# ielym/fastvision

Hardware: AMD Instinct MI355X
Metric: images/sec (640×640, bs=32/GPU) YOLOv3 train step, 1/2/4/8 MI355X (higher is better)
Workload: dtype bf16

## Files before the change

### fastvision_amd/csrc/conv_igemm.hip

```cpp
#include <stddef.h>
#include <stdlib.h>

#include "common.h"

namespace {

enum { EPI_STATS = 0, EPI_PLAIN = 1, EPI_HEAD = 2, EPI_BNACT = 3, EPI_BNB = 4 };
constexpr int MAX_TAPS = 10;

struct IgemmParams {
    const void* in;
    const void* wt;
    void* out;
    float* stats;
    int acc_rep, bnb_rep, ax_rep;
    long long* stats_acc;
    const float* bias;
    const float* scale;
    int act;
    const float* shift;
    int M, N, C;
    int OW, OHW;
    FastDiv div_ow, div_ohw;
    int in_img, in_row;
// ... 17 lines not shown
    const float *ax_scale, *ax_shift;
    int ax_pad, ax_res_pad, ax_H, ax_W;
    long long* ax_acc;
    long long* ax_zero;
    const float *ax_gamma, *ax_beta;
    float *ax_rm, *ax_rv;
    long long* ax_nbt;
    float ax_momentum, ax_eps;
    BnN ax_n;
    float *ax_save_mean, *ax_save_rstd, *ax_scale_out, *ax_shift_out;
    long long* stamps;
    int stamp_rows;
    int pt_tx, pt_ty, pt_H, pt_W;
    int pt_tiles, pt_tpb;
    FastDiv pt_div_tx, pt_div_img;
};

struct BnbCoef {
    float sc[8], sh[8], mu[8], rs[8];
};
__device__ __forceinline__ void bnb_load(const IgemmParams& p, int n, BnbCoef& k) {
#pragma unroll
    for (int e = 0; e < 8; ++e) {
        int c = n + e;
        c = c < p.N ? c : p.N - 1;
        c = c >= p.bnb_C ? c - p.bnb_C : c;
        k.sc[e] = p.bnb_scale[c]; k.sh[e] = p.bnb_shift[c]; k.mu[e] = p.bnb_mean[c]; k.rs[e] = p.bnb_rstd[c];
    }
}
template <int BN, int NT>
__device__ __forceinline__ float bnb_coef_at(const IgemmParams& p, int i, int n0) {
// ... 169 lines not shown
__device__ __forceinline__ void foreach_acc(Acc<float>& acc, int lane, F&& f) {
    const int r = lane & 31, h = lane >> 5;
#pragma unroll
    for (int mt = 0; mt < 2; ++mt)
#pragma unroll
        for (int nt = 0; nt < 2; ++nt)
#pragma unroll
            for (int e = 0; e < 16; ++e) f(mt * 32 + (e & 3) + 8 * (e >> 2) + 4 * h, nt * 32 + r, nt, acc.a[mt][nt][e]);
}

template <int N>
__device__ __forceinline__ void wait_vmcnt() {
    asm volatile("s_waitcnt vmcnt(%0)" ::"n"(N) : "memory");
}

template <typename T, int BM, int BN, int EPI, int NSTAGE, bool AX = false>
__global__ __launch_bounds__((BM / 64) * (BN / 64) * 64) void igemm_kernel(const IgemmParams p) {
    static_assert(!AX || (sizeof(T) == 2 && EPI == EPI_STATS), "the produced-operand form is the bf16 training forward of a 1x1 layer");
    constexpr int EPC = 16 / (int)sizeof(T);
    constexpr int BK = 8 * EPC;
    constexpr int WN = BN / 64;
    constexpr int NW = (BM / 64) * WN;
    constexpr int NT = NW * 64;
    static_assert(NW % 2 == 0, "the source swizzle assumes an even wave count");
    constexpr int A_BYTES = BM * 128, B_BYTES = BN * 128, STAGE = A_BYTES + B_BYTES;
    constexpr int A_ITERS = BM / (8 * NW), B_ITERS = BN / (8 * NW);
    constexpr bool IS_BF16 = sizeof(T) == 2;
    extern __shared__ __attribute__((aligned(16))) char smem[];

    const int tid = threadIdx.x, lane = tid & 63, w = tid >> 6;
    const int wr = w / WN, wc = w % WN;
    auto stamp = [&](int i) {
        if (p.stamps && tid == 0 && (int)blockIdx.x < p.stamp_rows) p.stamps[(int64_t)blockIdx.x * 8 + i] = wall_clock64();
    };
    stamp(0);

    const int nwg = gridDim.x, bid = blockIdx.x;
    const int xcd = bid & 7, xq = nwg >> 3, xr = nwg & 7;
    const int logical = (xcd < xr ? xcd * (xq + 1) : xr * (xq + 1) + (xcd - xr) * xq) + (bid >> 3);
    const int mblk = logical / p.nblocks, nblk = logical - mblk * p.nblocks;
    const int m0 = mblk * BM, n0 = nblk * BN;

    const T* a_ptr[A_ITERS];
    const T* b_ptr[B_ITERS];
    const int lrow = lane >> 3;
    const int sw = ((w & 1) << 2) + (lane >> 4);
    const int chunk = (lane & 7) ^ sw;
    const int tapsel = chunk >> 2;
    const int sub = p.halfrow ? (chunk & 3) : chunk;
#pragma unroll
    for (int i = 0; i < A_ITERS; ++i) {
        int m = m0 + (i * NW + w) * 8 + lrow;
        m = m < p.M ? m : p.M - 1;
        const uint32_t b = fd_div((uint32_t)m, p.div_ohw);
        const uint32_t rem = (uint32_t)m - b * (uint32_t)p.OHW;
        const uint32_t oy = fd_div(rem, p.div_ow);
// ... 7 lines not shown
        n = n < p.N ? n : p.N - 1;
        b_ptr[i] = (const T*)p.wt + (int64_t)n * p.C + sub * EPC;
    }

    constexpr bool USE_KTAB = BN >= 128;
    constexpr int COEF_BYTES = (EPI == EPI_BNB && IS_BF16 && BN >= 128) ? 4 * BN * 4 : 0;
    float* coef_tab = (float*)(smem + NSTAGE * STAGE);
    int* ktab = (int*)(smem + NSTAGE * STAGE + COEF_BYTES);
    constexpr int COEF_PER_THREAD = COEF_BYTES > 0 ? 4 * BN / NT : 0;
    float coef_v[COEF_PER_THREAD > 0 ? COEF_PER_THREAD : 1];
    if constexpr (COEF_BYTES > 0) {
#pragma unroll
        for (int j = 0; j < COEF_PER_THREAD; ++j) coef_v[j] = bnb_coef_at<BN, NT>(p, tid + j * NT, n0);
    }
    if constexpr (USE_KTAB) {
        const int nent = p.halfrow ? 2 * p.ktiles : p.ktiles;
        for (int e = tid; e < nent; e += NT) {
            int t, kk;
            if (p.halfrow) { t = e; kk = 0; }
            else if (p.ktaps) { kk = e / p.ktaps; t = e - kk * p.ktaps; }
            else { t = e / p.kt_per_tap; kk = e - t * p.kt_per_tap; }
            int tp = 0, tw = 0;
#pragma unroll
            for (int i = 0; i < MAX_TAPS; ++i)
                if (i == t) { tp = p.tap_pix[i]; tw = p.tap_w[i]; }
            ktab[2 * e] = tp * p.C + kk * BK;
            ktab[2 * e + 1] = tw * p.N * p.C + kk * BK;
        }
        __syncthreads();
    }
    stamp(6);
    int ld_tap = 0, ld_kk = 0;
    auto load_tile = [&](int kt, int stage) {
        char* sA = smem + stage * STAGE;
        char* sB = sA + A_BYTES;
        int aoff, boff;
        if constexpr (USE_KTAB) {
            const int e = p.halfrow ? 2 * kt + tapsel : kt;
            aoff = ktab[2 * e];
            boff = ktab[2 * e + 1];
        } else {
            const int t = p.halfrow ? ld_tap + tapsel : ld_tap;
            int tp = 0, tw = 0;
#pragma unroll
            for (int i = 0; i < MAX_TAPS; ++i)
                if (i == t) { tp = p.tap_pix[i]; tw = p.tap_w[i]; }
            aoff = tp * p.C + ld_kk * BK;
            boff = tw * p.N * p.C + ld_kk * BK;
            if (p.halfrow) ld_tap += 2;
            else if (++ld_kk == p.kt_per_tap) { ld_kk = 0; ++ld_tap; }
        }
#pragma unroll
        for (int i = 0; i < A_ITERS; ++i)
            __builtin_amdgcn_global_load_lds(GLB_PTR(a_ptr[i] + aoff), LDS_PTR(sA + (i * NW + w) * 1024), 16, 0, 0);
#pragma unroll
        for (int i = 0; i < B_ITERS; ++i)
            __builtin_amdgcn_global_load_lds(GLB_PTR(b_ptr[i] + boff), LDS_PTR(sB + (i * NW + w) * 1024), 16, 0, 0);
    };

    bf16x8 y_pre[8], a_pre[8];
    constexpr bool PREFETCH = (EPI == EPI_BNB || EPI == EPI_PLAIN) && sizeof(T) == 2;
// ... 1 lines not shown
        constexpr int CPR = BN / 8, RSTEP = NT / CPR;
        static_assert(BM * CPR / NT == 8, "the prefetch covers the whole store loop");
        const int cc = tid % CPR, r0 = tid / CPR;
        const int n = n0 + cc * 8;
#pragma unroll
        for (int j = 0; j < 8; ++j) {
            const int m = m0 + r0 + j * RSTEP;
            int64_t oi = 0;
            if (n < p.N && m < p.M) {
                int64_t pixel = m;
                if (!p.out_dense) {
                    const uint32_t b = fd_div((uint32_t)m, p.div_ohw);
                    const uint32_t rem = (uint32_t)m - b * (uint32_t)p.OHW;
                    const uint32_t oy = fd_div(rem, p.div_ow);
                    const uint32_t ox = rem - oy * (uint32_t)p.OW;
                    pixel = (int64_t)b * p.out_img + (int64_t)(oy * p.osy + p.ooy) * p.out_row + (ox * p.osx + p.oox);
                }
                oi = pixel * p.out_pitch + n;
            }
            if constexpr (EPI == EPI_BNB) y_pre[j] = ld_stream((const bf16_t*)p.bnb_y + oi);
            if (p.addend != nullptr) a_pre[j] = ld_stream((const bf16_t*)p.addend + oi);
        }
    }

    Acc<T> acc;
    if constexpr (sizeof(T) == 2) {
#pragma unroll
        for (int i = 0; i < 4; ++i)
#pragma unroll
            for (int j = 0; j < 4; ++j) acc.a[i][j] = f32x4{0.f, 0.f, 0.f, 0.f};
    } else {
// ... 51 lines not shown
        constexpr int S = decltype(set_tag)::value;
#pragma unroll
        for (int i = 0; i < A_ITERS; ++i) {
            ax_ry[S][i] = *(const bf16x8*)((const bf16_t*)p.ax_y + ax_yo[i] + kt * BK);
            if (ax_has_res) ax_rr[S][i] = *(const bf16x8*)((const bf16_t*)p.ax_res + ax_ro[i] + kt * BK);
        }
        if constexpr (!AXT) {
            const int c0 = kt * BK + chunk * 8;
            ax_csc[0] = *(const f32x4*)(p.ax_scale + c0); ax_csc[1] = *(const f32x4*)(p.ax_scale + c0 + 4);
            ax_csh[0] = *(const f32x4*)(p.ax_shift + c0); ax_csh[1] = *(const f32x4*)(p.ax_shift + c0 + 4);
        }
    };
    auto ax_step = [&](int kt, auto set_tag) {
        constexpr int S = decltype(set_tag)::value;
        if constexpr (AXS == 2) {
            if (kt + 1 < p.ktiles) {
                ax_load_raw(kt + 1, std::integral_constant<int, S ^ 1>{});
                if (ax_has_res) wait_vmcnt<2 * A_ITERS>();
                else wait_vmcnt<A_ITERS>();
            } else {
                wait_vmcnt<0>();
            }
        } else {
            wait_vmcnt<0>();
        }
        __builtin_amdgcn_sched_barrier(0);
        const uint32_t sAw = (uint32_t)(size_t)LDS_PTR(smem + st_cur * STAGE);
        f32x4 ax_sc[2], ax_sh[2];
        if constexpr (!AXT) {
            ax_sc[0] = ax_csc[0]; ax_sc[1] = ax_csc[1]; ax_sh[0] = ax_csh[0]; ax_sh[1] = ax_csh[1];
        } else {
// ... 29 lines not shown
                    if (f & 8u) {
                        *(bf16x8*)(q - zrow) = zero;
                        if (f & 2u) *(bf16x8*)(q - zrow - p.C) = zero;
                        if (f & 4u) *(bf16x8*)(q - zrow + p.C) = zero;
                    }
                    if (f & 16u) {
                        *(bf16x8*)(q + zrow) = zero;
                        if (f & 2u) *(bf16x8*)(q + zrow - p.C) = zero;
                        if (f & 4u) *(bf16x8*)(q + zrow + p.C) = zero;
                    }
                }
            }
        }
        asm volatile("s_waitcnt lgkmcnt(0)" ::: "memory");
        __builtin_amdgcn_s_barrier();
        if (kt + 1 < p.ktiles) {
            ax_issue_b(kt + 1, st_cur ^ 1);
            if constexpr (AXS == 1) ax_load_raw(kt + 1, std::integral_constant<int, 0>{});
        }
    };
    if constexpr (AX) {
        const int zp = p.ax_pad, rp = p.ax_res_pad;
        const uint32_t zW = (uint32_t)(p.ax_W + 2 * zp), zHW = (uint32_t)(p.ax_H + 2 * zp) * zW;
        const uint32_t rW = (uint32_t)(p.ax_W + 2 * rp), rHW = (uint32_t)(p.ax_H + 2 * rp) * rW;
#pragma unroll
        for (int i = 0; i < A_ITERS; ++i) {
            int m = m0 + (i * NW + w) * 8 + lrow;
            const bool live = m < p.M;
            m = live ? m : p.M - 1;
            const uint32_t b = fd_div((uint32_t)m, p.div_ohw);
            const uint32_t rem = (uint32_t)m - b * (uint32_t)p.OHW;
// ... 5 lines not shown
            ax_fl[i] = (live ? 1u : 0u) | (zp > 0 && live ? ((ox == 0 ? 2u : 0u) | (ox == (uint32_t)p.ax_W - 1 ? 4u : 0u) | (oy == 0 ? 8u : 0u) |
                                                           (oy == (uint32_t)p.ax_H - 1 ? 16u : 0u)) : 0u);
        }
        ax_load_raw(0, std::integral_constant<int, 0>{});
        if constexpr (AXT) {
            for (int c = tid; c < p.C; c += NT) ax_coef(c, logical == 0, ax_tab[c], ax_tab[p.C + c]);
            __syncthreads();
        }
        if (AXT && p.ax_acc != nullptr && logical == 0) {
            if (tid == 0 && p.ax_nbt) *p.ax_nbt += 1;
            fx_zero(p.ax_zero, p.C, p.ax_rep, tid, NT);
        }
        ax_issue_b(0, 0);
    } else {
        load_tile(0, 0);
        if (p.ktiles > 1) load_tile(1, 1);
    }
    stamp(1);
    for (int kt = 0; kt < p.ktiles; ++kt) {
        if constexpr (AX) {
            if (AXS == 1 || (kt & 1) == 0) ax_step(kt, std::integral_constant<int, 0>{});
            else ax_step(kt, std::integral_constant<int, AXS - 1>{});
            if (kt == 0) stamp(2);
        } else {
        if (kt == 0 && p.ktiles > 1) wait_vmcnt<LPT>();
        else wait_vmcnt<0>();
        __builtin_amdgcn_s_barrier();
        if (kt == 0) stamp(2);
        if (kt >= 1 && kt + 1 < p.ktiles) load_tile(kt + 1, st_cur ^ 1);
        }
        const char* sA = smem + st_cur * STAGE;
        const char* sB = sA + A_BYTES;
        st_cur ^= 1;
        if constexpr (IS_BF16) {
            const int r = lane & 15, g = lane >> 4, sr = (r >> 1) & 7;
            const char* pa = sA + (wr * 64 + r) * 128;
            const char* pb = sB + (wc * 64 + r) * 128;
#pragma unroll
            for (int ks = 0; ks < 2; ++ks) {
                const int co = ((ks * 4 + g) ^ sr) << 4;
                bf16x8 af[4], bfr[4];
#pragma unroll
                for (int t = 0; t < 4; ++t) {
                    af[t] = *(const bf16x8*)(pa + t * 16 * 128 + co);
// ... 111 lines not shown
                        if (p.stats_acc != nullptr) fx_atomic_add(fx_replica(p.stats_acc, p.N, p.acc_rep), p.N, which, n0 + col, s);
                        else *(p.stats + ((int64_t)mblk * 2 + which) * p.N + n0 + col) = s;
                    }
                }
                __syncthreads();
            }
        }
    }

    auto out_pixel = [&](int m) -> int64_t {
        if (p.out_dense) return m;
        const uint32_t b = fd_div((uint32_t)m, p.div_ohw);
        const uint32_t rem = (uint32_t)m - b * (uint32_t)p.OHW;
        const uint32_t oy = fd_div(rem, p.div_ow);
        const uint32_t ox = rem - oy * (uint32_t)p.OW;
        return (int64_t)b * p.out_img + (int64_t)(oy * p.osy + p.ooy) * p.out_row + (ox * p.osx + p.oox);
    };

    if constexpr (EPI == EPI_HEAD) {
        float* out = (float*)p.out;
        foreach_acc(acc, lane, [&](int row, int col, int, float v) {
            const int m = m0 + wrow0 + row, n = n0 + wcol0 + col;
            if (m < p.M && n < p.N) out[(int64_t)m * p.out_pitch + n] = v + p.bias[n];
        });
    } else if constexpr (!IS_BF16) {
        float* out = (float*)p.out;
        int64_t pix_cache = -1;
        int m_cache = -1;
        constexpr bool bnb = EPI == EPI_BNB;
        float b1[2] = {0.f, 0.f}, b2[2] = {0.f, 0.f}, ksc[2], ksh[2], kmu[2], krs[2];
        if constexpr (bnb) {
// ... 38 lines not shown
                    if (lane < 32) {
                        red[(0 * WMc + wr) * BN + wcol0 + i * 32 + lane] = b1[i];
                        red[(1 * WMc + wr) * BN + wcol0 + i * 32 + lane] = b2[i];
                    }
                }
                __syncthreads();
                if (w < BN / 32) {
                    const int which = lane >> 5, col = w * 32 + (lane & 31);
                    float t = 0.f;
#pragma unroll
                    for (int k = 0; k < WMc; ++k) t += red[(which * WMc + k) * BN + col];
                    const int n = n0 + col;
                    const int sub = n >= p.bnb_C ? 1 : 0, per = p.N > p.bnb_C ? 2 : 1;
                    if (n < p.N) {
                        if (p.bnb_acc != nullptr) fx_atomic_add(fx_replica(p.bnb_acc, p.bnb_C, p.bnb_rep), p.bnb_C, which, n - sub * p.bnb_C, t);
                        else *(p.bnb_part + (((int64_t)(p.bnb_row0 + mblk) * per + sub) * 2 + which) * p.bnb_C + (n - sub * p.bnb_C)) = t;
                    }
                }
            }
        }
    } else {
        constexpr int PITCH = BN * 2 + 16;
        if constexpr (EPI == EPI_BNB && COEF_BYTES == 0) {
            coef_tab = (float*)(smem + BM * PITCH);
            static_assert(4 * BN <= NT || EPI != EPI_BNB || COEF_BYTES > 0, "one table entry per thread");
            if (tid < 4 * BN) coef_v[0] = bnb_coef_at<BN, NT>(p, tid, n0);
        }
        {
            const int r = lane & 15, g = lane >> 4;
#pragma unroll
            for (int mt = 0; mt < 4; ++mt)
// ... 1 lines not shown
                for (int nt = 0; nt < 4; ++nt) {
                    f32x4 v = acc.a[mt][nt];
                    const int col = wcol0 + nt * 16 + 4 * g;
                    if constexpr (EPI == EPI_BNACT) {
#pragma unroll
                        for (int j = 0; j < 4; ++j) v[j] = bnact_f(p, v[j], n0 + col + j < p.N ? n0 + col + j : p.N - 1);
                    }
                    *(u32x2*)(smem + (wrow0 + mt * 16 + r) * PITCH + col * 2) = u32x2{cvt_pk_bf16(v[0], v[1]), cvt_pk_bf16(v[2], v[3])};
                }
        }
        if constexpr (EPI == EPI_BNB && COEF_BYTES == 0) {
            if (tid < 4 * BN) coef_tab[tid] = coef_v[0];
        }
        __syncthreads();
        stamp(4);
        store_tile_bf16<EPI, BM, BN, NT, PITCH>(p, smem, tid, n0, mblk, [&](int row) { const int m = m0 + row; return m < p.M ? out_pixel(m) : (int64_t)-1; },
                                                EPI == EPI_BNB ? y_pre : nullptr, PREFETCH ? a_pre : nullptr, coef_tab);
    }
    if constexpr (AX) {

    }
    stamp(5);
}

template <typename T, int BM, int BN, int EPI, int NSTAGE, bool AX = false>
int launch_one(const IgemmParams& p, hipStream_t s) {
    const int mblocks = cdiv(p.M, BM);
    IgemmParams q = p;
    q.nblocks = cdiv(p.N, BN);
    static const bool stamp_tiles = [] { const char* e = getenv("FVA_STAMP_IGEMM"); return e && atoi(e) != 0; }();
    q.stamps = stamp_tiles ? fva_debug_stamps_ptr() : nullptr;
    q.stamp_rows = stamp_tiles ? fva_debug_stamps_rows() : 0;
    constexpr int KTAB_MAX = 16384;
    const int nent = (p.halfrow ? 2 : 1) * p.ktiles;
    if (BN >= 128 && nent * 8 > KTAB_MAX) return fva_fail(FVA_ERR_ARG, "igemm: %d k-tiles exceed the offset table (%d)", p.ktiles, KTAB_MAX / 8);
    const int ktab_bytes = BN >= 128 ? (nent * 8 > 4096 ? (nent * 8 + 255) & ~255 : 4096) : 0;
    constexpr int coef_bytes = (EPI == EPI_BNB && sizeof(T) == 2 && BN >= 128) ? 4 * BN * 4 : 0;
    const int smem = NSTAGE * (BM + BN) * 128 + ktab_bytes + coef_bytes;
    static bool attr_done = false;
    if (!attr_done) {
        (void)hipFuncSetAttribute((const void*)igemm_kernel<T, BM, BN, EPI, NSTAGE, AX>, hipFuncAttributeMaxDynamicSharedMemorySize,
                                  NSTAGE * (BM + BN) * 128 + (BN >= 128 ? KTAB_MAX : 0) + coef_bytes);
        attr_done = true;
    }
    hipLaunchKernelGGL((igemm_kernel<T, BM, BN, EPI, NSTAGE, AX>), dim3(mblocks * q.nblocks), dim3((BM / 64) * (BN / 64) * 64), smem, s, q);
    FVA_LAUNCH_CHECK("igemm_kernel");
    fva_note_kernel(AX ? (BM == 128 ? "igemm128ax" : "igemm256x64ax") : (BM == 128 ? "igemm128" : "igemm256x64"));
    return FVA_OK;
}


struct PconvGeom {
    static constexpr int PH = 10, PW = 34, PW_RCP = 1928;
    static constexpr int OY = 8, OX = 32;
    static constexpr int TH = 8, TW_LOG2 = 5;
    static constexpr int NA = 4, NGRP = 4;
    static constexpr int MIN_CS = 32;
    static constexpr bool STATS = true, BNB_LOOPS = true;
    static constexpr const char *LABEL = "pconv", *KERNEL = "pconv_kernel";
    static __device__ __forceinline__ int frag_pix(int w, int a, int r16) { return (2 * w + (a >> 1)) * PW + (a & 1) * 16 + r16; }
// ... 299 lines not shown
    p.pt_ty = cdiv(H, G::TH);
    p.pt_div_tx = make_fastdiv(p.pt_tx);
    p.pt_div_img = make_fastdiv(p.pt_tx * p.pt_ty);
    for (int t = 0; t < 9; ++t) p.tap_w[t] = flip ? 8 - t : t;
    return G::template launch_form<EPI>(p, patch_tiles<G>(B, H, W), s);
}

struct Igemm8Diag {
    long long* stamps;
    int stamp_rows;
};

#ifndef FVA_EPI_STAMPS
#define FVA_EPI_STAMPS 0
#endif
template <int EPI>
__global__ __launch_bounds__(512) void igemm8_kernel(const IgemmParams p, const Igemm8Diag sk) {
    constexpr int MT = 8;
    constexpr int WM = 16 * MT;
    constexpr int BM = 2 * WM, BN = 256, NT = 512, BK = 64;
    constexpr int HALF = 128 * 128, BUF = 4 * HALF;
    constexpr int EPI_BYTES = BM * (BN * 2 + 16);
    constexpr int TAB0 = EPI_BYTES > 2 * BUF ? EPI_BYTES : 2 * BUF;
    extern __shared__ __attribute__((aligned(16))) char smem[];
    const int tid = threadIdx.x, lane = tid & 63, w = tid >> 6;
    const int wr = w >> 2, wc = w & 3;
    auto stamp = [&](int i) {
        if (sk.stamps && tid == 0 && (int)blockIdx.x < sk.stamp_rows) {
            sk.stamps[(int64_t)blockIdx.x * 8 + i] = wall_clock64();
            sk.stamps[(int64_t)blockIdx.x * 8 + 4 + i] = clock64();
        }
    };
#if !FVA_EPI_STAMPS
    stamp(0);
#endif

    const int nwg = gridDim.x, bid = blockIdx.x;
    const int xcd = bid & 7, xq = nwg >> 3, xr = nwg & 7;
    const int logical = (xcd < xr ? xcd * (xq + 1) : xr * (xq + 1) + (xcd - xr) * xq) + (bid >> 3);
    const int KT = p.ktiles;

    int* ktab = (int*)(smem + TAB0);
    for (int e = tid; e < KT; e += NT) {
        int t, kk;
        if (p.ktaps) { kk = e / p.ktaps; t = e - kk * p.ktaps; }
        else { t = e / p.kt_per_tap; kk = e - t * p.kt_per_tap; }
        int tp = 0, tw = 0;
#pragma unroll
        for (int i = 0; i < MAX_TAPS; ++i)
            if (i == t) { tp = p.tap_pix[i]; tw = p.tap_w[i]; }
        ktab[2 * e] = tp * p.C + kk * BK;
        ktab[2 * e + 1] = tw * p.N * p.C + kk * BK;
    }

    const int lrow = lane >> 3;
    const int chunk = (lane & 7) ^ (((w & 1) << 2) + (lane >> 4));
    const int r = lane & 15, g = lane >> 4, sr = (r >> 1) & 7;
    const int co0 = (g ^ sr) << 4, co1 = ((4 + g) ^ sr) << 4;
    const int a_row = (wr * 64 + r) * 128, b_row = (wc * 32 + r) * 128;

    {
        const int tile = logical, kt0 = 0, kt1 = KT;
        const int mblk = tile / p.nblocks, nblk = tile - mblk * p.nblocks;
        const int m0 = mblk * BM, n0 = nblk * BN;
        __syncthreads();
        float* coef_tab = (float*)(smem + TAB0 + 4096);
        if constexpr (EPI == EPI_BNB) bnb_fill_lds<BN, NT>(p, coef_tab, tid, n0);

        uint32_t a_off[2][2], b_off[2][2];
#pragma unroll
        for (int h = 0; h < 2; ++h)
#pragma unroll
            for (int i = 0; i < 2; ++i) {
                const int rh = (i * 8 + w) * 8 + lrow;
                int m = m0 + (rh >> 6) * WM + h * 64 + (rh & 63);
                m = m < p.M ? m : p.M - 1;
                const uint32_t b = fd_div((uint32_t)m, p.div_ohw);
                const uint32_t rem = (uint32_t)m - b * (uint32_t)p.OHW;
                const uint32_t oy = fd_div(rem, p.div_ow);
// ... 154 lines not shown
                    if (n0 + col < p.N) {
                        if (p.stats_acc != nullptr) fx_atomic_add(fx_replica(p.stats_acc, p.N, p.acc_rep), p.N, which, n0 + col, s);
                        else *(p.stats + ((int64_t)mblk * 2 + which) * p.N + n0 + col) = s;
                    }
                }
                __syncthreads();
            }
        }

        auto out_pixel = [&](int m) -> int64_t {
            if (p.out_dense) return m;
            const uint32_t b = fd_div((uint32_t)m, p.div_ohw);
            const uint32_t rem = (uint32_t)m - b * (uint32_t)p.OHW;
            const uint32_t oy = fd_div(rem, p.div_ow);
            const uint32_t ox = rem - oy * (uint32_t)p.OW;
            return (int64_t)b * p.out_img + (int64_t)(oy * p.osy + p.ooy) * p.out_row + (ox * p.osx + p.oox);
        };
        constexpr int PITCH = BN * 2 + 16;
#if FVA_EPI_STAMPS
        stamp(1);
#endif
#pragma unroll
        for (int mi = 0; mi < MT; ++mi)
#pragma unroll
            for (int ni = 0; ni < 4; ++ni) {
                f32x4 v = acc[mi][ni];
                if constexpr (EPI == EPI_BNACT) {
#pragma unroll
                    for (int j = 0; j < 4; ++j) v[j] = bnact_f(p, v[j], n0 + col_e + ni * 16 + j);
                }
                *(u32x2*)(smem + (row_e + mi * 16) * PITCH + (col_e + ni * 16) * 2) = u32x2{cvt_pk_bf16(v[0], v[1]), cvt_pk_bf16(v[2], v[3])};
            }
        __syncthreads();
#if FVA_EPI_STAMPS
        stamp(2);
#endif
        store_tile_bf16<EPI, BM, BN, NT, PITCH>(p, smem, tid_e, n0, mblk, [&](int row) { const int m = m0 + row; return m < p.M ? out_pixel(m) : (int64_t)-1; },
                                                nullptr, nullptr, EPI == EPI_BNB ? coef_tab : nullptr);
    }
    stamp(3);
}

constexpr int IGEMM8_SMEM = 256 * (256 * 2 + 16) + 4096 + 4096;

inline bool igemm8_enabled() {
    static bool v = [] {
        const char* e = getenv("FVA_IGEMM8");
        return !e || atoi(e) != 0;
    }();
    return v;
}
inline bool use_igemm8(int dtype, int64_t M, int N, int C, int ntaps, int64_t in_pixels) {
    if (!igemm8_enabled() || dtype != FVA_BF16 || N % 256 || C % 64) return false;
    if (in_pixels * C * 2 >= (1ll << 31) || (int64_t)(ntaps + 1) * N * C * 2 >= (1ll << 31)) return false;
    const int64_t ktiles = (int64_t)ntaps * (C / 64), tiles = (int64_t)cdiv(M, 256) * (N / 256);
    if (ktiles > 496 || ktiles < 8) return false;
    if (tiles < 128) return false;
    static const int min_kt = [] { const char* e = getenv("FVA_IGEMM8_MINKT"); return e ? atoi(e) : 16; }();
    return ktiles >= min_kt || tiles <= 256;
}

long long* g_stamps = nullptr;
int g_stamp_rows = 0;

template <int EPI>
int launch_igemm8(const IgemmParams& p, hipStream_t s) {
    IgemmParams q = p;
    q.nblocks = p.N / 256;
    const int tiles = cdiv(p.M, 256) * q.nblocks;
    static bool attr_done = false;
    if (!attr_done) {
        (void)hipFuncSetAttribute((const void*)igemm8_kernel<EPI>, hipFuncAttributeMaxDynamicSharedMemorySize, IGEMM8_SMEM);
        attr_done = true;
    }
    Igemm8Diag sk{};
    sk.stamps = g_stamps;
    sk.stamp_rows = g_stamp_rows;
    hipLaunchKernelGGL((igemm8_kernel<EPI>), dim3(tiles), dim3(512), IGEMM8_SMEM, s, q, sk);
    fva_note_kernel("igemm8");
    FVA_LAUNCH_CHECK("igemm8_kernel");
    return FVA_OK;
}

inline bool wide_tile(int N) { return N >= 128; }

inline int tile_bm(int , int , int N) { return wide_tile(N) ? 128 : 256; }

template <int EPI>
int launch_igemm(int dtype, const IgemmParams& p, hipStream_t s) {
    if (dtype == FVA_BF16) {
        if constexpr (EPI != EPI_HEAD) {
            if (!p.halfrow && use_igemm8(dtype, p.M, p.N, p.C, p.ktiles / p.kt_per_tap, (int64_t)(p.M / p.OHW + 1) * p.in_img))
                return launch_igemm8<EPI>(p, s);
        }
        return wide_tile(p.N) ? launch_one<bf16_t, 128, 128, EPI, 2>(p, s) : launch_one<bf16_t, 256, 64, EPI, 2>(p, s);
    }
    return wide_tile(p.N) ? launch_one<float, 128, 128, EPI, 2>(p, s) : launch_one<float, 256, 64, EPI, 2>(p, s);
}

int check_desc(const fva_conv_desc* d, const char* who) {
    if (!d) return fva_fail(FVA_ERR_ARG, "%s: null descriptor", who);
    if (d->dtype != FVA_F32 && d->dtype != FVA_BF16) return fva_fail(FVA_ERR_ARG, "%s: bad dtype %d", who, d->dtype);
    if (!((d->ksize == 1 && d->stride == 1) || (d->ksize == 3 && (d->stride == 1 || d->stride == 2))))
        return fva_fail(FVA_ERR_ARG, "%s: unsupported ksize/stride %d/%d", who, d->ksize, d->stride);
    if (d->B <= 0 || d->H <= 0 || d->W <= 0 || d->Cin <= 0 || d->Cout <= 0)
        return fva_fail(FVA_ERR_ARG, "%s: non-positive size", who);
    if (d->stride == 2 && ((d->H | d->W) & 1)) return fva_fail(FVA_ERR_ARG, "%s: stride 2 needs even H, W", who);
    if (d->in_pad < d->ksize / 2) return fva_fail(FVA_ERR_ARG, "%s: in_pad %d < %d", who, d->in_pad, d->ksize / 2);
    if ((int64_t)d->B * (d->H + 2) * (d->W + 2) >= (1ll << 31)) return fva_fail(FVA_ERR_ARG, "%s: too many pixels", who);
    return FVA_OK;
}

// ... 467 lines not shown
    int rc = setup_fwd(d, p, "fva_head_fwd");
    if (rc) return rc;
    if (d->ksize != 1) return fva_fail(FVA_ERR_ARG, "fva_head_fwd: ksize must be 1");
    if (!x || !w_fwd || !bias || !out) return fva_fail(FVA_ERR_ARG, "fva_head_fwd: null pointer");
    p.in = x;
    p.wt = w_fwd;
    p.out = out;
    p.bias = bias;
    FvaProfileSpan span(0 | (d->ksize << 8), 2.0 * p.M * (double)d->Cout * d->Cin * d->ksize * d->ksize, (hipStream_t)stream);
    return launch_igemm<EPI_HEAD>(d->dtype, p, (hipStream_t)stream);
}

static int dgrad_launch_rows(const fva_conv_desc* d, int64_t m, int n, int c, int ntaps, int64_t in_pixels) {
    if (!halfrow_mode(d->dtype, c) && use_igemm8(d->dtype, m, n, c, ntaps, in_pixels)) return cdiv(m, 256);
    return cdiv(m, tile_bm(d->dtype, (int)m, n));
}

int32_t fva_conv_dgrad_stat_rows(const fva_conv_desc* d) {
    if (!d || check_desc(d, "fva_conv_dgrad_stat_rows")) return 0;
    const int k = d->ksize, s = d->stride;
    const int OH = (d->H - 1) / s + 1, OW = (d->W - 1) / s + 1;
    const int64_t in_pixels = (int64_t)(d->B + 1) * (OH + 2 * d->dy_pad) * (OW + 2 * d->dy_pad);
    if (use_pconv(d->dtype, k, s, d->Cout, d->Cin, d->H, d->W)) return patch_tiles<PconvGeom>(d->B, d->H, d->W);
    if (s == 1) return dgrad_launch_rows(d, (int64_t)d->B * d->H * d->W, d->Cin, d->Cout, k * k, in_pixels);
    const int64_t mq = (int64_t)d->B * (d->H / 2) * (d->W / 2);
    if (use_pdgrad2(d->dtype, k, s, d->Cout, d->Cin)) return patch_tiles<Pdgrad2Geom>(d->B, d->H, d->W);
    if (dgrad_paired(d->dtype, k, s, d->Cin, d->Cout)) {
        int rows = 0;
        for (int py = 0; py < 2; ++py) rows += 2 * dgrad_launch_rows(d, mq, 2 * d->Cin, d->Cout, py == 0 ? 2 : 4, in_pixels);
        return rows;
// ... 71 lines not shown
        return f ? launch_patch<Pdgrad2Geom, EPI_BNB>(p, d->B, d->H, d->W, false, (hipStream_t)stream) : launch_patch<Pdgrad2Geom, EPI_PLAIN>(p, d->B, d->H, d->W, false, (hipStream_t)stream);
    }
    if (dgrad_paired(d->dtype, k, s, d->Cin, d->Cout)) {
        p.M = d->B * JH * JW;
        p.N = 2 * d->Cin;
        p.OW = JW;
        p.OHW = JH * JW;
        p.div_ow = make_fastdiv(p.OW);
        p.div_ohw = make_fastdiv(p.OHW);
        p.y0 = p.x0 = 0;
        p.out_dense = 0;
        p.out_img = d->H * d->W;
        p.out_row = d->W;
        p.osy = p.osx = 2;
        p.oox = 0;
        for (int py = 0; py < 2; ++py) {
            int nt = 0;
            const int nky = py == 0 ? 1 : 2;
            const int kys[2] = {py == 0 ? 1 : 0, 2};
            const int yos[2] = {py == 0 ? d->dy_pad : d->dy_pad + 1, d->dy_pad};
            for (int a = 0; a < nky; ++a)
                for (int dxo = 0; dxo < 2; ++dxo) {
                    p.tap_pix[nt] = yos[a] * p.in_row + d->dy_pad + dxo;
                    p.tap_w[nt] = kys[a] * 2 + dxo;
                    ++nt;
                }
            p.tap_w[nt] = 0;
            finish_taps(p, nt, d->dtype);
            if (p.halfrow) return fva_fail(FVA_ERR_ARG, "fva_conv_dgrad: paired stride-2 path needs Cout >= 64");
            p.ooy = py;
            rc = f ? launch_igemm<EPI_BNB>(d->dtype, p, (hipStream_t)stream) : launch_igemm<EPI_PLAIN>(d->dtype, p, (hipStream_t)stream);
            if (rc) return rc;
            p.bnb_row0 += dgrad_launch_rows(d, p.M, p.N, p.C, nt, in_pixels);
        }
        return FVA_OK;
    }
    p.M = d->B * JH * JW;
    p.OW = JW;
    p.OHW = JH * JW;
    p.div_ow = make_fastdiv(p.OW);
    p.div_ohw = make_fastdiv(p.OHW);
    p.y0 = p.x0 = 0;
    p.out_dense = 0;
    p.out_img = d->H * d->W;
    p.out_row = d->W;
    p.osy = p.osx = 2;
    for (int py = 0; py < 2; ++py)
        for (int px = 0; px < 2; ++px) {
            int khs[2], yo[2], nky, kws[2], xo[2], nkx;
            if (py == 0) { nky = 1; khs[0] = 1; yo[0] = d->dy_pad; }
            else { nky = 2; khs[0] = 0; yo[0] = d->dy_pad + 1; khs[1] = 2; yo[1] = d->dy_pad; }
            if (px == 0) { nkx = 1; kws[0] = 1; xo[0] = d->dy_pad; }
            else { nkx = 2; kws[0] = 0; xo[0] = d->dy_pad + 1; kws[1] = 2; xo[1] = d->dy_pad; }
            int nt = 0;
            for (int a = 0; a < nky; ++a)
                for (int b = 0; b < nkx; ++b) {
                    p.tap_pix[nt] = yo[a] * p.in_row + xo[b];
                    p.tap_w[nt] = khs[a] * 3 + kws[b];
                    ++nt;
                }
            p.tap_w[nt] = 9;
            finish_taps(p, nt, d->dtype);
            p.ooy = py;
            p.oox = px;
            rc = f ? launch_igemm<EPI_BNB>(d->dtype, p, (hipStream_t)stream) : launch_igemm<EPI_PLAIN>(d->dtype, p, (hipStream_t)stream);
            if (rc) return rc;
            p.bnb_row0 += dgrad_launch_rows(d, p.M, p.N, p.C, nt, in_pixels);
        }
    return FVA_OK;
}

}
```

Baseline: 1131.

## Fuse stride-2 dgrad phase-class launches into one multi-class igemm launch

```diff
diff --git a/fastvision_amd/csrc/conv_igemm.hip b/fastvision_amd/csrc/conv_igemm.hip
--- a/fastvision_amd/csrc/conv_igemm.hip
+++ b/fastvision_amd/csrc/conv_igemm.hip
@@ -7,6 +7,15 @@
 
 enum { EPI_STATS = 0, EPI_PLAIN = 1, EPI_HEAD = 2, EPI_BNACT = 3, EPI_BNB = 4 };
 constexpr int MAX_TAPS = 10;
+constexpr int MAX_CLS = 4, CLS_TAPS = 4;
+
+struct IgemmClass {
+    int tap_pix[CLS_TAPS], tap_w[CLS_TAPS];
+    int ktiles, ktaps;
+    int ooy, oox;
+    int bnb_row0;
+    int blk0, nblk;
+};
 
 struct IgemmParams {
     const void* in;
@@ -55,7 +64,24 @@
     int pt_tx, pt_ty, pt_H, pt_W;
     int pt_tiles, pt_tpb;
     FastDiv pt_div_tx, pt_div_img;
+    int ncls;
+    IgemmClass cls[MAX_CLS];
 };
+
+__device__ __forceinline__ IgemmClass igemm_class_of(const IgemmParams& p, int& bid, int& nwg) {
+    IgemmClass c = p.cls[0];
+#pragma unroll
+    for (int i = 1; i < MAX_CLS; ++i)
+        if (i < p.ncls && bid >= p.cls[i].blk0) c = p.cls[i];
+    bid -= c.blk0;
+    nwg = c.nblk;
+    return c;
+}
+__device__ __forceinline__ void igemm_class_tap(const IgemmClass& c, int t, int& tp, int& tw) {
+#pragma unroll
+    for (int i = 0; i < CLS_TAPS; ++i)
+        if (i == t) { tp = c.tap_pix[i]; tw = c.tap_w[i]; }
+}
 
 struct BnbCoef {
     float sc[8], sh[8], mu[8], rs[8];
@@ -255,8 +281,9 @@
     asm volatile("s_waitcnt vmcnt(%0)" ::"n"(N) : "memory");
 }
 
-template <typename T, int BM, int BN, int EPI, int NSTAGE, bool AX = false>
+template <typename T, int BM, int BN, int EPI, int NSTAGE, bool AX = false, bool MULTI = false>
 __global__ __launch_bounds__((BM / 64) * (BN / 64) * 64) void igemm_kernel(const IgemmParams p) {
+    static_assert(!MULTI || (!AX && (EPI == EPI_PLAIN || EPI == EPI_BNB)), "several classes per launch: the stride-2 data gradients");
     static_assert(!AX || (sizeof(T) == 2 && EPI == EPI_STATS), "the produced-operand form is the bf16 training forward of a 1x1 layer");
     constexpr int EPC = 16 / (int)sizeof(T);
     constexpr int BK = 8 * EPC;
@@ -276,11 +303,24 @@
     };
     stamp(0);
 
-    const int nwg = gridDim.x, bid = blockIdx.x;
+    int nwg = gridDim.x, bid = blockIdx.x;
+    IgemmClass cl = {};
+    if constexpr (MULTI) cl = igemm_class_of(p, bid, nwg);
+    const int KT = MULTI ? cl.ktiles : p.ktiles, ktaps = MULTI ? cl.ktaps : p.ktaps;
+    const int ooy = MULTI ? cl.ooy : p.ooy, oox = MULTI ? cl.oox : p.oox;
+    auto tap_at = [&](int t, int& tp, int& tw) {
+        if constexpr (MULTI) igemm_class_tap(cl, t, tp, tw);
+        else {
+#pragma unroll
+            for (int i = 0; i < MAX_TAPS; ++i)
+                if (i == t) { tp = p.tap_pix[i]; tw = p.tap_w[i]; }
+        }
+    };
     const int xcd = bid & 7, xq = nwg >> 3, xr = nwg & 7;
     const int logical = (xcd < xr ? xcd * (xq + 1) : xr * (xq + 1) + (xcd - xr) * xq) + (bid >> 3);
     const int mblk = logical / p.nblocks, nblk = logical - mblk * p.nblocks;
     const int m0 = mblk * BM, n0 = nblk * BN;
+    const int srow = MULTI ? cl.bnb_row0 + mblk : mblk;
 
     const T* a_ptr[A_ITERS];
     const T* b_ptr[B_ITERS];
@@ -318,16 +358,14 @@
         for (int j = 0; j < COEF_PER_THREAD; ++j) coef_v[j] = bnb_coef_at<BN, NT>(p, tid + j * NT, n0);
     }
     if constexpr (USE_KTAB) {
-        const int nent = p.halfrow ? 2 * p.ktiles : p.ktiles;
+        const int nent = p.halfrow ? 2 * KT : KT;
         for (int e = tid; e < nent; e += NT) {
             int t, kk;
             if (p.halfrow) { t = e; kk = 0; }
-            else if (p.ktaps) { kk = e / p.ktaps; t = e - kk * p.ktaps; }
+            else if (ktaps) { kk = e / ktaps; t = e - kk * ktaps; }
             else { t = e / p.kt_per_tap; kk = e - t * p.kt_per_tap; }
             int tp = 0, tw = 0;
-#pragma unroll
-            for (int i = 0; i < MAX_TAPS; ++i)
-                if (i == t) { tp = p.tap_pix[i]; tw = p.tap_w[i]; }
+            tap_at(t, tp, tw);
             ktab[2 * e] = tp * p.C + kk * BK;
             ktab[2 * e + 1] = tw * p.N * p.C + kk * BK;
         }
@@ -346,9 +384,7 @@
         } else {
             const int t = p.halfrow ? ld_tap + tapsel : ld_tap;
             int tp = 0, tw = 0;
-#pragma unroll
-            for (int i = 0; i < MAX_TAPS; ++i)
-                if (i == t) { tp = p.tap_pix[i]; tw = p.tap_w[i]; }
+            tap_at(t, tp, tw);
             aoff = tp * p.C + ld_kk * BK;
             boff = tw * p.N * p.C + ld_kk * BK;
             if (p.halfrow) ld_tap += 2;
@@ -380,7 +416,7 @@
                     const uint32_t rem = (uint32_t)m - b * (uint32_t)p.OHW;
                     const uint32_t oy = fd_div(rem, p.div_ow);
                     const uint32_t ox = rem - oy * (uint32_t)p.OW;
-                    pixel = (int64_t)b * p.out_img + (int64_t)(oy * p.osy + p.ooy) * p.out_row + (ox * p.osx + p.oox);
+                    pixel = (int64_t)b * p.out_img + (int64_t)(oy * p.osy + ooy) * p.out_row + (ox * p.osx + oox);
                 }
                 oi = pixel * p.out_pitch + n;
             }
@@ -462,7 +498,7 @@
     auto ax_step = [&](int kt, auto set_tag) {
         constexpr int S = decltype(set_tag)::value;
         if constexpr (AXS == 2) {
-            if (kt + 1 < p.ktiles) {
+            if (kt + 1 < KT) {
                 ax_load_raw(kt + 1, std::integral_constant<int, S ^ 1>{});
                 if (ax_has_res) wait_vmcnt<2 * A_ITERS>();
                 else wait_vmcnt<A_ITERS>();
@@ -522,7 +558,7 @@
         }
         asm volatile("s_waitcnt lgkmcnt(0)" ::: "memory");
         __builtin_amdgcn_s_barrier();
-        if (kt + 1 < p.ktiles) {
+        if (kt + 1 < KT) {
             ax_issue_b(kt + 1, st_cur ^ 1);
             if constexpr (AXS == 1) ax_load_raw(kt + 1, std::integral_constant<int, 0>{});
         }
@@ -558,20 +594,20 @@
         ax_issue_b(0, 0);
     } else {
         load_tile(0, 0);
-        if (p.ktiles > 1) load_tile(1, 1);
+        if (KT > 1) load_tile(1, 1);
     }
     stamp(1);
-    for (int kt = 0; kt < p.ktiles; ++kt) {
+    for (int kt = 0; kt < KT; ++kt) {
         if constexpr (AX) {
             if (AXS == 1 || (kt & 1) == 0) ax_step(kt, std::integral_constant<int, 0>{});
             else ax_step(kt, std::integral_constant<int, AXS - 1>{});
             if (kt == 0) stamp(2);
         } else {
-        if (kt == 0 && p.ktiles > 1) wait_vmcnt<LPT>();
+        if (kt == 0 && KT > 1) wait_vmcnt<LPT>();
         else wait_vmcnt<0>();
         __builtin_amdgcn_s_barrier();
         if (kt == 0) stamp(2);
-        if (kt >= 1 && kt + 1 < p.ktiles) load_tile(kt + 1, st_cur ^ 1);
+        if (kt >= 1 && kt + 1 < KT) load_tile(kt + 1, st_cur ^ 1);
         }
         const char* sA = smem + st_cur * STAGE;
         const char* sB = sA + A_BYTES;
@@ -713,7 +749,7 @@
         const uint32_t rem = (uint32_t)m - b * (uint32_t)p.OHW;
         const uint32_t oy = fd_div(rem, p.div_ow);
         const uint32_t ox = rem - oy * (uint32_t)p.OW;
-        return (int64_t)b * p.out_img + (int64_t)(oy * p.osy + p.ooy) * p.out_row + (ox * p.osx + p.oox);
+        return (int64_t)b * p.out_img + (int64_t)(oy * p.osy + ooy) * p.out_row + (ox * p.osx + oox);
     };
 
     if constexpr (EPI == EPI_HEAD) {
@@ -782,7 +818,7 @@
                     const int sub = n >= p.bnb_C ? 1 : 0, per = p.N > p.bnb_C ? 2 : 1;
                     if (n < p.N) {
                         if (p.bnb_acc != nullptr) fx_atomic_add(fx_replica(p.bnb_acc, p.bnb_C, p.bnb_rep), p.bnb_C, which, n - sub * p.bnb_C, t);
-                        else *(p.bnb_part + (((int64_t)(p.bnb_row0 + mblk) * per + sub) * 2 + which) * p.bnb_C + (n - sub * p.bnb_C)) = t;
+                        else *(p.bnb_part + (((int64_t)(p.bnb_row0 + srow) * per + sub) * 2 + which) * p.bnb_C + (n - sub * p.bnb_C)) = t;
                     }
                 }
             }
@@ -814,7 +850,7 @@
         }
         __syncthreads();
         stamp(4);
-        store_tile_bf16<EPI, BM, BN, NT, PITCH>(p, smem, tid, n0, mblk, [&](int row) { const int m = m0 + row; return m < p.M ? out_pixel(m) : (int64_t)-1; },
+        store_tile_bf16<EPI, BM, BN, NT, PITCH>(p, smem, tid, n0, srow, [&](int row) { const int m = m0 + row; return m < p.M ? out_pixel(m) : (int64_t)-1; },
                                                 EPI == EPI_BNB ? y_pre : nullptr, PREFETCH ? a_pre : nullptr, coef_tab);
     }
     if constexpr (AX) {
@@ -823,11 +859,21 @@
     stamp(5);
 }
 
-template <typename T, int BM, int BN, int EPI, int NSTAGE, bool AX = false>
+inline int place_classes(IgemmParams& q, int tiles) {
+    for (int i = 0; i < q.ncls; ++i) {
+        q.cls[i].blk0 = i * tiles;
+        q.cls[i].nblk = tiles;
+    }
+    return q.ncls * tiles;
+}
+
+template <typename T, int BM, int BN, int EPI, int NSTAGE, bool AX = false, bool MULTI = false>
 int launch_one(const IgemmParams& p, hipStream_t s) {
     const int mblocks = cdiv(p.M, BM);
     IgemmParams q = p;
     q.nblocks = cdiv(p.N, BN);
+    int grid = mblocks * q.nblocks;
+    if constexpr (MULTI) grid = place_classes(q, grid);
     static const bool stamp_tiles = [] { const char* e = getenv("FVA_STAMP_IGEMM"); return e && atoi(e) != 0; }();
     q.stamps = stamp_tiles ? fva_debug_stamps_ptr() : nullptr;
     q.stamp_rows = stamp_tiles ? fva_debug_stamps_rows() : 0;
@@ -839,11 +885,11 @@
     const int smem = NSTAGE * (BM + BN) * 128 + ktab_bytes + coef_bytes;
     static bool attr_done = false;
     if (!attr_done) {
-        (void)hipFuncSetAttribute((const void*)igemm_kernel<T, BM, BN, EPI, NSTAGE, AX>, hipFuncAttributeMaxDynamicSharedMemorySize,
+        (void)hipFuncSetAttribute((const void*)igemm_kernel<T, BM, BN, EPI, NSTAGE, AX, MULTI>, hipFuncAttributeMaxDynamicSharedMemorySize,
                                   NSTAGE * (BM + BN) * 128 + (BN >= 128 ? KTAB_MAX : 0) + coef_bytes);
         attr_done = true;
     }
-    hipLaunchKernelGGL((igemm_kernel<T, BM, BN, EPI, NSTAGE, AX>), dim3(mblocks * q.nblocks), dim3((BM / 64) * (BN / 64) * 64), smem, s, q);
+    hipLaunchKernelGGL((igemm_kernel<T, BM, BN, EPI, NSTAGE, AX, MULTI>), dim3(grid), dim3((BM / 64) * (BN / 64) * 64), smem, s, q);
     FVA_LAUNCH_CHECK("igemm_kernel");
     fva_note_kernel(AX ? (BM == 128 ? "igemm128ax" : "igemm256x64ax") : (BM == 128 ? "igemm128" : "igemm256x64"));
     return FVA_OK;
@@ -1173,8 +1219,9 @@
 #ifndef FVA_EPI_STAMPS
 #define FVA_EPI_STAMPS 0
 #endif
-template <int EPI>
+template <int EPI, bool MULTI = false>
 __global__ __launch_bounds__(512) void igemm8_kernel(const IgemmParams p, const Igemm8Diag sk) {
+    static_assert(!MULTI || EPI == EPI_PLAIN || EPI == EPI_BNB, "several classes per launch: the stride-2 data gradients");
     constexpr int MT = 8;
     constexpr int WM = 16 * MT;
     constexpr int BM = 2 * WM, BN = 256, NT = 512, BK = 64;
@@ -1194,20 +1241,26 @@
     stamp(0);
 #endif
 
-    const int nwg = gridDim.x, bid = blockIdx.x;
+    int nwg = gridDim.x, bid = blockIdx.x;
+    IgemmClass cl = {};
+    if constexpr (MULTI) cl = igemm_class_of(p, bid, nwg);
     const int xcd = bid & 7, xq = nwg >> 3, xr = nwg & 7;
     const int logical = (xcd < xr ? xcd * (xq + 1) : xr * (xq + 1) + (xcd - xr) * xq) + (bid >> 3);
-    const int KT = p.ktiles;
+    const int KT = MULTI ? cl.ktiles : p.ktiles, ktaps = MULTI ? cl.ktaps : p.ktaps;
+    const int ooy = MULTI ? cl.ooy : p.ooy, oox = MULTI ? cl.oox : p.oox;
 
     int* ktab = (int*)(smem + TAB0);
     for (int e = tid; e < KT; e += NT) {
         int t, kk;
-        if (p.ktaps) { kk = e / p.ktaps; t = e - kk * p.ktaps; }
+        if (ktaps) { kk = e / ktaps; t = e - kk * ktaps; }
         else { t = e / p.kt_per_tap; kk = e - t * p.kt_per_tap; }
         int tp = 0, tw = 0;
-#pragma unroll
-        for (int i = 0; i < MAX_TAPS; ++i)
-            if (i == t) { tp = p.tap_pix[i]; tw = p.tap_w[i]; }
+        if constexpr (MULTI) igemm_class_tap(cl, t, tp, tw);
+        else {
+#pragma unroll
+            for (int i = 0; i < MAX_TAPS; ++i)
+                if (i == t) { tp = p.tap_pix[i]; tw = p.tap_w[i]; }
+        }
         ktab[2 * e] = tp * p.C + kk * BK;
         ktab[2 * e + 1] = tw * p.N * p.C + kk * BK;
     }
@@ -1222,6 +1275,7 @@
         const int tile = logical, kt0 = 0, kt1 = KT;
         const int mblk = tile / p.nblocks, nblk = tile - mblk * p.nblocks;
         const int m0 = mblk * BM, n0 = nblk * BN;
+        const int srow = MULTI ? cl.bnb_row0 + mblk : mblk;
         __syncthreads();
         float* coef_tab = (float*)(smem + TAB0 + 4096);
         if constexpr (EPI == EPI_BNB) bnb_fill_lds<BN, NT>(p, coef_tab, tid, n0);
@@ -1406,7 +1460,7 @@
             const uint32_t rem = (uint32_t)m - b * (uint32_t)p.OHW;
             const uint32_t oy = fd_div(rem, p.div_ow);
             const uint32_t ox = rem - oy * (uint32_t)p.OW;
-            return (int64_t)b * p.out_img + (int64_t)(oy * p.osy + p.ooy) * p.out_row + (ox * p.osx + p.oox);
+            return (int64_t)b * p.out_img + (int64_t)(oy * p.osy + ooy) * p.out_row + (ox * p.osx + oox);
         };
         constexpr int PITCH = BN * 2 + 16;
 #if FVA_EPI_STAMPS
@@ -1427,7 +1481,7 @@
 #if FVA_EPI_STAMPS
         stamp(2);
 #endif
-        store_tile_bf16<EPI, BM, BN, NT, PITCH>(p, smem, tid_e, n0, mblk, [&](int row) { const int m = m0 + row; return m < p.M ? out_pixel(m) : (int64_t)-1; },
+        store_tile_bf16<EPI, BM, BN, NT, PITCH>(p, smem, tid_e, n0, srow, [&](int row) { const int m = m0 + row; return m < p.M ? out_pixel(m) : (int64_t)-1; },
                                                 nullptr, nullptr, EPI == EPI_BNB ? coef_tab : nullptr);
     }
     stamp(3);
@@ -1455,20 +1509,21 @@
 long long* g_stamps = nullptr;
 int g_stamp_rows = 0;
 
-template <int EPI>
+template <int EPI, bool MULTI = false>
 int launch_igemm8(const IgemmParams& p, hipStream_t s) {
     IgemmParams q = p;
     q.nblocks = p.N / 256;
-    const int tiles = cdiv(p.M, 256) * q.nblocks;
+    int tiles = cdiv(p.M, 256) * q.nblocks;
+    if constexpr (MULTI) tiles = place_classes(q, tiles);
     static bool attr_done = false;
     if (!attr_done) {
-        (void)hipFuncSetAttribute((const void*)igemm8_kernel<EPI>, hipFuncAttributeMaxDynamicSharedMemorySize, IGEMM8_SMEM);
+        (void)hipFuncSetAttribute((const void*)igemm8_kernel<EPI, MULTI>, hipFuncAttributeMaxDynamicSharedMemorySize, IGEMM8_SMEM);
         attr_done = true;
     }
     Igemm8Diag sk{};
     sk.stamps = g_stamps;
     sk.stamp_rows = g_stamp_rows;
-    hipLaunchKernelGGL((igemm8_kernel<EPI>), dim3(tiles), dim3(512), IGEMM8_SMEM, s, q, sk);
+    hipLaunchKernelGGL((igemm8_kernel<EPI, MULTI>), dim3(tiles), dim3(512), IGEMM8_SMEM, s, q, sk);
     fva_note_kernel("igemm8");
     FVA_LAUNCH_CHECK("igemm8_kernel");
     return FVA_OK;
@@ -1488,6 +1543,15 @@
         return wide_tile(p.N) ? launch_one<bf16_t, 128, 128, EPI, 2>(p, s) : launch_one<bf16_t, 256, 64, EPI, 2>(p, s);
     }
     return wide_tile(p.N) ? launch_one<float, 128, 128, EPI, 2>(p, s) : launch_one<float, 256, 64, EPI, 2>(p, s);
+}
+
+template <int EPI>
+int launch_igemm_classes(int dtype, const IgemmParams& p, bool use8, hipStream_t s) {
+    if (dtype == FVA_BF16) {
+        if (use8) return launch_igemm8<EPI, true>(p, s);
+        return wide_tile(p.N) ? launch_one<bf16_t, 128, 128, EPI, 2, false, true>(p, s) : launch_one<bf16_t, 256, 64, EPI, 2, false, true>(p, s);
+    }
+    return wide_tile(p.N) ? launch_one<float, 128, 128, EPI, 2, false, true>(p, s) : launch_one<float, 256, 64, EPI, 2, false, true>(p, s);
 }
 
 int check_desc(const fva_conv_desc* d, const char* who) {
@@ -1985,6 +2049,71 @@
 static int dgrad_launch_rows(const fva_conv_desc* d, int64_t m, int n, int c, int ntaps, int64_t in_pixels) {
     if (!halfrow_mode(d->dtype, c) && use_igemm8(d->dtype, m, n, c, ntaps, in_pixels)) return cdiv(m, 256);
     return cdiv(m, tile_bm(d->dtype, (int)m, n));
+}
+
+struct S2Class {
+    int tap_pix[CLS_TAPS], tap_w[CLS_TAPS];
+    int nt, ooy, oox;
+};
+
+static bool s2_one_launch() {
+    static const bool v = [] { const char* e = getenv("FVA_DGRAD_S2_LAUNCHES"); return !e || atoi(e) != 4; }();
+    return v;
+}
+
+static int launch_s2_classes(const fva_conv_desc* d, IgemmParams& p, const S2Class* sc, int ncls, int zero_tap, bool fused, int64_t in_pixels,
+                             hipStream_t stream) {
+    const bool halfrow = halfrow_mode(d->dtype, p.C);
+    int row0[MAX_CLS], use8[MAX_CLS], rows = 0;
+    bool same = true;
+    for (int i = 0; i < ncls; ++i) {
+        row0[i] = rows;
+        rows += dgrad_launch_rows(d, p.M, p.N, p.C, sc[i].nt, in_pixels);
+        use8[i] = !halfrow && use_igemm8(d->dtype, p.M, p.N, p.C, sc[i].nt, in_pixels) ? 1 : 0;
+        same = same && use8[i] == use8[0];
+    }
+    if (same && !halfrow && ncls > 1 && s2_one_launch()) {
+        int order[MAX_CLS];
+        for (int i = 0; i < ncls; ++i) {
+            int j = i;
+            for (; j > 0 && sc[order[j - 1]].nt < sc[i].nt; --j) order[j] = order[j - 1];
+            order[j] = i;
+        }
+        int ktmax = 0;
+        for (int j = 0; j < ncls; ++j) {
+            const S2Class& c = sc[order[j]];
+            IgemmClass& k = p.cls[j];
+            for (int t = 0; t < CLS_TAPS; ++t) {
+                k.tap_pix[t] = t < c.nt ? c.tap_pix[t] : 0;
+                k.tap_w[t] = t < c.nt ? c.tap_w[t] : zero_tap;
+            }
+            finish_taps(p, c.nt, d->dtype);
+            k.ktiles = p.ktiles;
+            k.ktaps = p.ktaps;
+            k.ooy = c.ooy;
+            k.oox = c.oox;
+            k.bnb_row0 = row0[order[j]];
+            ktmax = k.ktiles > ktmax ? k.ktiles : ktmax;
+        }
+        p.ncls = ncls;
+        p.ktiles = ktmax;
+        p.bnb_row0 = 0;
+        return fused ? launch_igemm_classes<EPI_BNB>(d->dtype, p, use8[0] != 0, stream) : launch_igemm_classes<EPI_PLAIN>(d->dtype, p, use8[0] != 0, stream);
+    }
+    for (int i = 0; i < ncls; ++i) {
+        for (int t = 0; t < sc[i].nt; ++t) {
+            p.tap_pix[t] = sc[i].tap_pix[t];
+            p.tap_w[t] = sc[i].tap_w[t];
+        }
+        p.tap_w[sc[i].nt] = zero_tap;
+        finish_taps(p, sc[i].nt, d->dtype);
+        p.ooy = sc[i].ooy;
+        p.oox = sc[i].oox;
+        p.bnb_row0 = row0[i];
+        const int rc = fused ? launch_igemm<EPI_BNB>(d->dtype, p, stream) : launch_igemm<EPI_PLAIN>(d->dtype, p, stream);
+        if (rc) return rc;
+    }
+    return FVA_OK;
 }
 
 int32_t fva_conv_dgrad_stat_rows(const fva_conv_desc* d) {
@@ -2086,6 +2215,8 @@
         p.out_row = d->W;
         p.osy = p.osx = 2;
         p.oox = 0;
+        if (halfrow_mode(d->dtype, p.C)) return fva_fail(FVA_ERR_ARG, "fva_conv_dgrad: paired stride-2 path needs Cout >= 64");
+        S2Class sc[2];
         for (int py = 0; py < 2; ++py) {
             int nt = 0;
             const int nky = py == 0 ? 1 : 2;
@@ -2093,19 +2224,15 @@
             const int yos[2] = {py == 0 ? d->dy_pad : d->dy_pad + 1, d->dy_pad};
             for (int a = 0; a < nky; ++a)
                 for (int dxo = 0; dxo < 2; ++dxo) {
-                    p.tap_pix[nt] = yos[a] * p.in_row + d->dy_pad + dxo;
-                    p.tap_w[nt] = kys[a] * 2 + dxo;
+                    sc[py].tap_pix[nt] = yos[a] * p.in_row + d->dy_pad + dxo;
+                    sc[py].tap_w[nt] = kys[a] * 2 + dxo;
                     ++nt;
                 }
-            p.tap_w[nt] = 0;
-            finish_taps(p, nt, d->dtype);
-            if (p.halfrow) return fva_fail(FVA_ERR_ARG, "fva_conv_dgrad: paired stride-2 path needs Cout >= 64");
-            p.ooy = py;
-            rc = f ? launch_igemm<EPI_BNB>(d->dtype, p, (hipStream_t)stream) : launch_igemm<EPI_PLAIN>(d->dtype, p, (hipStream_t)stream);
-            if (rc) return rc;
-            p.bnb_row0 += dgrad_launch_rows(d, p.M, p.N, p.C, nt, in_pixels);
-        }
-        return FVA_OK;
+            sc[py].nt = nt;
+            sc[py].ooy = py;
+            sc[py].oox = 0;
+        }
+        return launch_s2_classes(d, p, sc, 2, 0, f != nullptr, in_pixels, (hipStream_t)stream);
     }
     p.M = d->B * JH * JW;
     p.OW = JW;
@@ -2117,6 +2244,7 @@
     p.out_img = d->H * d->W;
     p.out_row = d->W;
     p.osy = p.osx = 2;
+    S2Class sc[4];
     for (int py = 0; py < 2; ++py)
         for (int px = 0; px < 2; ++px) {
             int khs[2], yo[2], nky, kws[2], xo[2], nkx;
@@ -2124,22 +2252,19 @@
             else { nky = 2; khs[0] = 0; yo[0] = d->dy_pad + 1; khs[1] = 2; yo[1] = d->dy_pad; }
             if (px == 0) { nkx = 1; kws[0] = 1; xo[0] = d->dy_pad; }
             else { nkx = 2; kws[0] = 0; xo[0] = d->dy_pad + 1; kws[1] = 2; xo[1] = d->dy_pad; }
+            S2Class& c = sc[py * 2 + px];
             int nt = 0;
             for (int a = 0; a < nky; ++a)
                 for (int b = 0; b < nkx; ++b) {
-                    p.tap_pix[nt] = yo[a] * p.in_row + xo[b];
-                    p.tap_w[nt] = khs[a] * 3 + kws[b];
+                    c.tap_pix[nt] = yo[a] * p.in_row + xo[b];
+                    c.tap_w[nt] = khs[a] * 3 + kws[b];
                     ++nt;
                 }
-            p.tap_w[nt] = 9;
-            finish_taps(p, nt, d->dtype);
-            p.ooy = py;
-            p.oox = px;
-            rc = f ? launch_igemm<EPI_BNB>(d->dtype, p, (hipStream_t)stream) : launch_igemm<EPI_PLAIN>(d->dtype, p, (hipStream_t)stream);
-            if (rc) return rc;
-            p.bnb_row0 += dgrad_launch_rows(d, p.M, p.N, p.C, nt, in_pixels);
-        }
-    return FVA_OK;
-}
-
-}
+            c.nt = nt;
+            c.ooy = py;
+            c.oox = px;
+        }
+    return launch_s2_classes(d, p, sc, 4, 9, f != nullptr, in_pixels, (hipStream_t)stream);
+}
+
+}
```

Result: no change. 1129 (-0.2%).
